# cisco/thor

Measured on AMD Instinct MI355X. Metric: encoder Mpixels/s at fixed qp, bit-exact recon vs ref, higher is better.
Workload: dtype u8

## Files before the change

### include/thor_hip.h

```cpp
#ifndef THOR_HIP_H
#define THOR_HIP_H
#include <stddef.h>
#include <stdint.h>
#ifdef __cplusplus
extern "C" {
#endif

struct thor_encoder_info;
void encode_frame_lbd(struct thor_encoder_info* encoder_info);
void encode_frame_hbd(struct thor_encoder_info* encoder_info);

typedef struct thor_hip_params {
  int width, height, qp;
  int bitdepth, input_bitdepth;
  float frame_rate;
  float lambda_coeffI, lambda_coeffP;
  float early_skip_thr;
  int enable_tb_split, enable_pb_split, max_num_ref, HQperiod;
  int num_reorder_pics, interp_ref;
  int dqpP, dqpI;
  float mqpP;
  int intra_period, intra_rdo, encoder_speed;
  int deblocking, cdef, clpf, use_block_contexts, enable_bipred;
  int cfl_intra, cfl_inter;
// ... 57 lines not shown
  int frame_type;
  int qp;
  int num_bits;
  int num_ref;
  int ref_array[4];
  int ref_frame_num[4];
  int has_sse;
  unsigned long long sse[3];
  double psnr[3];
} thor_hip_frame_stats;
int thor_hip_frame_stats_count(const thor_hip_encoder* e, int stream);
int thor_hip_get_frame_stats(const thor_hip_encoder* e, int stream, int i, thor_hip_frame_stats* out);
int thor_hip_report(const thor_hip_encoder* e, int stream, char* buf, size_t n);
int thor_hip_stat_line(const thor_hip_encoder* e, int stream, int num_frames, char* buf, size_t n);

void thor_hip_read_prof(thor_hip_encoder* e, long long out[32]);

int thor_hip_sad_batch(const uint8_t* org, int w, int h, const uint8_t* ref_plane, int plane_w, int plane_h,
                       int rstride, int bx, int by, const int* cand, int n, uint32_t* out);
int thor_hip_interp_luma(const uint8_t* ref_plane, int plane_w, int plane_h, int rstride, int pad, int bx, int by,
                         int w, int h, const int16_t* mv, int n, int bipred, uint8_t* out);
int thor_hip_code_tu_batch(const uint8_t* org, const uint8_t* pred, int size, int qp, int coeff_type, int fast, int n,
                           int16_t* coefq, uint8_t* rec, int* cbp);
typedef struct thor_hip_cell {
  int16_t mv0x, mv0y, mv1x, mv1y;
  uint8_t mode, size, tbpb, cbp;
  int8_t ref0, ref1, dir;
  uint8_t pad;
} thor_hip_cell;
int thor_hip_deblock_frame(uint8_t* yuv, int width, int height, int qp, const thor_hip_cell* cells);

int thor_hip_sad_batch_hbd(const uint16_t* org, int w, int h, const uint16_t* ref_plane, int plane_w, int plane_h,
                           int rstride, int bx, int by, const int* cand, int n, uint32_t* out);
int thor_hip_interp_luma_hbd(const uint16_t* ref_plane, int plane_w, int plane_h, int rstride, int pad, int bx, int by,
                             int w, int h, const int16_t* mv, int n, int bipred, int bitdepth, uint16_t* out);
int thor_hip_code_tu_batch_hbd(const uint16_t* org, const uint16_t* pred, int size, int qp, int coeff_type, int fast, int n,
                               int bitdepth, int16_t* coefq, uint16_t* rec, int* cbp);
int thor_hip_deblock_frame_hbd(uint16_t* yuv, int width, int height, int qp, int bitdepth, const thor_hip_cell* cells);

int thor_hip_kat_intra(const void* plane, int width, int height, int stride, int bitdepth, int size, int tb_split, int n, const int* par,
                       const void* rblocks, void* out);
int thor_hip_kat_inter_yuv(const void* yuv, int width, int height, int bitdepth, int size, int n, const int* par, const int16_t* mv, void* out);
int thor_hip_kat_average(const void* a, const void* b, int size, int bitdepth, int n, void* out);
int thor_hip_kat_cfl(const void* y, void* uv, const void* ry, int n_luma, int bitdepth, int n);
int thor_hip_kat_cdef_dir(const void* blocks, int bitdepth, int n, int* dir, int* var);
int thor_hip_kat_cdef_filter(const void* plane, int width, int height, int stride, int bitdepth, int bsize, int n, const int* par, void* out);
int thor_hip_kat_cdef_frame(int n_jobs, const void* rec_yuv, const void* org_yuv, const uint8_t* mode, int width, int height, int bitdepth, const int* qp,
                            const int* speed, const int* cdef_bits, int8_t* dir, int* var, int* fb_compact, unsigned long long* mse, int* result, int* fb_sel, void* out_yuv);
int thor_hip_kat_clpf(const void* rec_yuv, const void* org_yuv, int width, int height, int bitdepth, int qp, const thor_hip_cell* cells,
                      const int* strength, int fb_log2, const uint8_t* fb_on, uint32_t* stats, void* out_yuv);
int thor_hip_kat_interpolate(const void* yuv0, const void* yuv1, int width, int height, int bitdepth, void* out_yuv);

int thor_hip_kat_motion_estimate(const void* cur, const void* ref, int width, int height, int bitdepth, int n, const int* par, const double* lambda,
                                 const int16_t* cand, int ncand_total, int* out);
int thor_hip_kat_motion_estimate_bi(const void* cur, const void* ref0, const void* ref1, int width, int height, int bitdepth, int n, const int* par,
                                    const double* lambda, const int16_t* cand, int* out, int16_t* list_out);
int thor_hip_kat_early_skip(const int* chroma, const void* org, const void* pred, const int* size, const int* qp, const float* thr, int bitdepth, int n, int* out);
int thor_hip_kat_coeff_syntax(int n, const int* par, const int16_t* coef, int words, uint32_t* buf_single, uint32_t* buf_team, int* out);
int thor_hip_kat_block_syntax(int n, const int* par, const int16_t* pool, int npool, int words, uint32_t* buf_coop, uint32_t* buf_single, int* out);
// ... 17 lines not shown
```

### thor_amd/__init__.py

```python
from .binding import (ThorParams, Encoder, FrameLayout, lib, lib_path, load_config, sad_batch, interp_luma, code_tu_batch, deblock_frame,
                      frame_sse, frame_sse_depth, kat_depth_up, kat_depth_down, layout_bytes, kat_layout_in,
                      kat_layout_out, build_native, REPO_ROOT)

__all__ = ['ThorParams', 'Encoder', 'FrameLayout', 'lib', 'lib_path', 'load_config', 'sad_batch', 'interp_luma', 'code_tu_batch', 'deblock_frame',
           'frame_sse', 'frame_sse_depth', 'kat_depth_up', 'kat_depth_down', 'layout_bytes', 'kat_layout_in', 'kat_layout_out', 'build_native', 'REPO_ROOT']
```

### thor_amd/binding.py

```python
import ctypes as C
import os
import subprocess
import numpy as np

REPO_ROOT = os.path.dirname(os.path.dirname(os.path.abspath(__file__)))
_LIB = None


def lib_path():
    return os.environ.get('THOR_HIP_LIB') or os.path.join(REPO_ROOT, 'thor_amd', 'libthor_hip.so')


HIPCC_FLAGS = ['--offload-arch=gfx950', '-O3', '-std=c++17', '-ffp-contract=off', '-fno-strict-aliasing', '-fPIC', '-pthread']
NATIVE_SOURCES = ['thor_hip.cpp', 'thor_hip_lat.cpp', 'thor_hip_wide.cpp', 'thor_hip_katbits.cpp']


def build_native(force=False):
    csrc = os.path.join(REPO_ROOT, 'thor_amd', 'csrc')
    out = os.path.join(REPO_ROOT, 'thor_amd', 'libthor_hip.so')
    hdrs = [os.path.join(csrc, f) for f in os.listdir(csrc)]
    hdrs += [os.path.join(REPO_ROOT, 'include', f) for f in os.listdir(os.path.join(REPO_ROOT, 'include'))]
    newest = max(os.path.getmtime(h) for h in hdrs)
    if force or not os.path.exists(out) or os.path.getmtime(out) < newest:
        hipcc = '/opt/rocm/bin/hipcc' if os.path.exists('/opt/rocm/bin/hipcc') else 'hipcc'
# ... 341 lines not shown
    else:
        rc = lib().thor_hip_interp_luma(_vp(ref_padded), pic_w, pic_h, ref_padded.shape[1], pad, bx, by, w, h, _vp(mvs), len(mvs),
                                        bipred, _vp(out))
    if rc:
        raise RuntimeError(f'thor_hip_interp_luma rc={rc}')
    return out


def code_tu_batch(org, pred, qp, coeff_type, fast, bitdepth=8):
    T = _pix(bitdepth)
    org = np.ascontiguousarray(org, dtype=T); pred = np.ascontiguousarray(pred, dtype=T)
    n, size = org.shape[0], org.shape[1]
    q = min(size, 16)
    coefq = np.zeros((n, q, q), dtype=np.int16); rec = np.zeros_like(org); cbp = np.zeros(n, dtype=np.int32)
    if bitdepth > 8:
        rc = lib().thor_hip_code_tu_batch_hbd(_vp(org), _vp(pred), size, qp, coeff_type, fast, n, bitdepth, _vp(coefq), _vp(rec), _vp(cbp))
    else:
        rc = lib().thor_hip_code_tu_batch(_vp(org), _vp(pred), size, qp, coeff_type, fast, n, _vp(coefq), _vp(rec), _vp(cbp))
    if rc:
        raise RuntimeError(f'thor_hip_code_tu_batch rc={rc}')
    return coefq, rec, cbp


def deblock_frame(yuv, width, height, qp, cells, bitdepth=8):
    yuv = np.ascontiguousarray(yuv, dtype=_pix(bitdepth)).copy()
    cells = np.ascontiguousarray(cells, dtype=np.uint8)
    assert yuv.size == width * height * 3 // 2 and cells.size == (width // 4) * (height // 4) * 16
    if bitdepth > 8:
        rc = lib().thor_hip_deblock_frame_hbd(_vp(yuv), width, height, qp, bitdepth, _vp(cells))
    else:
        rc = lib().thor_hip_deblock_frame(_vp(yuv), width, height, qp, _vp(cells))
    if rc:
        raise RuntimeError(f'thor_hip_deblock_frame rc={rc}')
    return yuv


def _kat(name, *args):
    fn = getattr(lib(), name)
    fn.restype = C.c_int
    rc = fn(*args)
    if rc:
        raise RuntimeError(f'{name} rc={rc}')


def kat_intra(plane, size, par, bitdepth=8, rblocks=None):
    T = _pix(bitdepth)
# ... 205 lines not shown
```

### thor_amd/csrc/hip_kat.h

```cpp
#pragma once
#include "tk_kat_bits.h"
namespace tk {
template <typename PIX>
__global__ __launch_bounds__(64) void k_kat_sad(const PIX* org, int w, int h, const PIX* refp, int rstride, int bx, int by, const int* cand, int n,
                                               uint32_t* out) {
  const Team t = mk_team((int)threadIdx.x, 64);
  struct KC { const PIX* p; int dx, dy; };
  MeWin win;
  win.on = 0; win.w32 = nullptr; win.ox = win.oy = win.Ww = win.Wh = win.pitch = 0;
  auto cnd = [&](int c) -> KC {
    KC x;
    x.dx = cand[2 * c]; x.dy = cand[2 * c + 1];
    x.p = refp + (size_t)(by + x.dy) * rstride + bx + x.dx;
    return x;
  };
  seg_sads<SP_GLOBAL>(t, n, org, w, rstride, w, h, win, cnd, [&](int c, const KC&, int sad, int mine) { if (mine) out[c] = (uint32_t)sad; });
}
template <typename PIX>
__global__ __launch_bounds__(64) void k_kat_interp(const PIX* ref0, int rstride, int pic_w, int pic_h, int bx, int by, int w, int h,
                                                  const int16_t* mv, int bipred, int bitdepth, PIX* out) {
  const Team t = mk_team((int)threadIdx.x, 64);
  const int i = blockIdx.x;
  pred_luma<SP_GLOBAL>(t, out + (size_t)i * w * h, w, ref0 + (size_t)by * rstride + bx, rstride, w, h, mk_mv(mv[2 * i], mv[2 * i + 1]), 0,
            bipred, pic_w, pic_h, bx, by, bitdepth);
}
template <typename PIX>
__global__ __launch_bounds__(64) void k_kat_tu(const PIX* org, const PIX* pred, int size, int qp, int coeff_type, int fast, int bitdepth,
                                              int16_t* coefq, PIX* rec, int* cbp) {
  __shared__ XformWs xf;
  __shared__ XformTabs tabs;
  __shared__ int16_t cq[256];
  const Team t = mk_team((int)threadIdx.x, 64, tabs.izz);
  xf.prof = nullptr;
  xf.tabs = &tabs;
  xform_tables_fill(&tabs, (int)threadIdx.x, 64);
  t.sync();
  const int i = blockIdx.x, qs = size < 16 ? size : 16;
  const size_t o = (size_t)i * size * size;
  int c = code_tu(t, &xf, org + o, size, pred + o, size, rec + o, size, size, qp, coeff_type, fast, cq, bitdepth);
  for (int k = threadIdx.x; k < qs * qs; k += 64) coefq[(size_t)i * qs * qs + k] = cq[k];
  if (threadIdx.x == 0) cbp[i] = c;
}

template <typename PIX>
__global__ __launch_bounds__(64) void k_kat_intra(const PIX* plane, int stride, int bitdepth, int size, int tb_split, const int* par, const PIX* rblocks,
                                                 PIX* out) {
  __shared__ IntraEdge<PIX> edge;
  const Team t = mk_team((int)threadIdx.x, 64);
  const int it = blockIdx.x;
  const int* q = par + 7 * it;
  const int cbs = tb_split ? 2 * size : size;
  const PIX* rblock = tb_split ? rblocks + (size_t)it * cbs * cbs + q[5] * cbs + q[6] : nullptr;
  make_edges<SP_GLOBAL>(t, &edge, plane + (size_t)q[0] * stride + q[1], stride, rblock, cbs, q[5], q[6], q[0], q[1], size, q[2], q[3], tb_split, bitdepth);
  pred_intra<SP_GLOBAL>(t, &edge, q[0] + q[5], q[1] + q[6], size, out + (size_t)it * size * size, size, q[4], bitdepth);
}
template <typename PIX>
__global__ __launch_bounds__(kWgThreads, (sizeof(PIX) == 1 ? (int)kOcc : 2)) void k_kat_inter_yuv(Plane3<PIX> ref, int width, int height, int bitdepth, int size, const int* par, const int16_t* mv, PIX* out) {
  const Team t = mk_team((int)threadIdx.x, 64);
  const int it = blockIdx.x;
  const int* q = par + 5 * it;
  mv_t m[4];
  for (int k = 0; k < 4; k++) m[k] = mk_mv(mv[(it * 4 + k) * 2], mv[(it * 4 + k) * 2 + 1]);
  PIX* o = out + (size_t)it * (size * size * 3 / 2);
  pred_inter_yuv<SP_GLOBAL>(t, ref, o, o + size * size, o + size * size * 5 / 4, q[0], q[1], size, size, size, m, q[2], width, height, q[3], q[4], bitdepth);
// ... 159 lines not shown
  const size_t px = (size_t)n * size * size;
  const int qs = size < 16 ? size : 16;
  DevBuf<PIX> d_org(px, org), d_pred(px, pred), d_rec(px);
  DevBuf<int16_t> d_cq((size_t)n * qs * qs);
  DevBuf<int> d_cbp(n);
  hipLaunchKernelGGL(k_kat_tu<PIX>, dim3(n), dim3(64), 0, g_stream, d_org, d_pred, size, qp, coeff_type, fast, bitdepth, d_cq, d_rec,
                     d_cbp);
  HIPCHECK(hipGetLastError());
  backend::d2h(coefq, d_cq, (size_t)n * qs * qs * 2);
  backend::d2h(rec, d_rec, px * sizeof(PIX));
  backend::d2h(cbp, d_cbp, (size_t)n * 4);
  return 0;
}
extern "C" int thor_hip_code_tu_batch(const uint8_t* org, const uint8_t* pred, int size, int qp, int coeff_type, int fast, int n,
                                      int16_t* coefq, uint8_t* rec, int* cbp) {
  return kat_code_tu_batch<uint8_t>(org, pred, size, qp, coeff_type, fast, n, 8, coefq, rec, cbp);
}
extern "C" int thor_hip_code_tu_batch_hbd(const uint16_t* org, const uint16_t* pred, int size, int qp, int coeff_type, int fast, int n,
                                          int bitdepth, int16_t* coefq, uint16_t* rec, int* cbp) {
  if (bitdepth < 9 || bitdepth > 12) return 1;
  return kat_code_tu_batch<uint16_t>(org, pred, size, qp, coeff_type, fast, n, bitdepth, coefq, rec, cbp);
}

template <typename PIX> static int kat_deblock_frame(PIX* yuv, int width, int height, int qp, int bitdepth, const thor_hip_cell* cells) {
  static_assert(sizeof(thor_hip_cell) == sizeof(DbCell), "thor_hip_cell must mirror tk::DbCell");
  if (!yuv || !cells || width % 8 || height % 8 || width < 16 || height < 16 || qp < 0 || qp > 51) return 1;
  if (!ensure_init_any()) return 3;
  DevFrame<PIX> f;
  f.alloc(width, height, 0);
  DevBuf<DbCell> d_cells((size_t)(width / 4) * (height / 4), (const DbCell*)cells);
  upload_yuv(f, yuv, width, height);
  FrameJob<PIX> J;
  memset(&J, 0, sizeof(J));
  J.cfg.width = width; J.cfg.height = height; J.cfg.bitdepth = bitdepth;
  J.qp = qp; J.rec = f.p; J.cells = d_cells; J.cell_stride = width / 4;
  DevBuf<FrameJob<PIX>> d_job(1, &J);
  backend::run_deblock<PIX>(d_job, &J, 1);
  backend::dev_sync();
  download_yuv(f, yuv, width, height);
  f.release();
  return 0;
}
extern "C" int thor_hip_deblock_frame(uint8_t* yuv, int width, int height, int qp, const thor_hip_cell* cells) {
  return kat_deblock_frame<uint8_t>(yuv, width, height, qp, 8, cells);
}
extern "C" int thor_hip_deblock_frame_hbd(uint16_t* yuv, int width, int height, int qp, int bitdepth, const thor_hip_cell* cells) {
// ... 508 lines not shown
```

### thor_amd/csrc/tk_block_rd.h

```cpp
#pragma once
#include "tk_block_ctx.h"

namespace tk {
template <typename PIX> struct SsdT { typedef unsigned long long type; };
template <> struct SsdT<uint8_t> { typedef unsigned type; };
TK_DEV unsigned udot4_u8(unsigned a, unsigned b, unsigned c) {
#if TK_HOST
  for (int k = 0; k < 4; k++) c += ((a >> (8 * k)) & 0xffu) * ((b >> (8 * k)) & 0xffu);
  return c;
#else
  return __builtin_amdgcn_udot4(a, b, c, false);
#endif
}
TK_DEV unsigned udot2_u16(unsigned a, unsigned b, unsigned c) {
#if TK_HOST
  return c + (a & 0xffffu) * (b & 0xffffu) + (a >> 16) * (b >> 16);
#else
  typedef unsigned short __attribute__((ext_vector_type(2))) u16x2;
  u16x2 x, y;
  __builtin_memcpy(&x, &a, 4); __builtin_memcpy(&y, &b, 4);
  return __builtin_amdgcn_udot2(x, y, c, false);
#endif
}
template <int SP, typename PIX, int NW> TK_DEV unsigned ssd_rows(const Team t, const PIX* a_, int as, const PIX* b_, int bs, int w, int h) {
// ... 218 lines not shown
  pc->ssd_y = (long long)ssd;
  const int coeff_type = (p.mode == M_INTRA) << 1;
  int bits = 0;
  if (!tb_split) {
    pc->ybits[0] = cbp_y ? coeff_bits_team<SP_LDS>(t, ws->coef_y, size, coeff_type) : 0;
    bits = pc->ybits[0];
  } else {
    const int qy = size / 2 < kMaxQuant ? size / 2 : kMaxQuant;
    for (int tu = 0; tu < 4; tu++) {
      pc->ybits[tu] = ((cbp_y >> (3 - tu)) & 1) ? coeff_bits_team<SP_LDS>(t, ws->coef_y + tu * qy * qy, size / 2, coeff_type) : 0;
      bits += pc->ybits[tu];
    }
  }
  pc->have_ybits = 1;
  unsigned long long lb = (ssd >> (J.cfg.bitdepth * 2 - 16)) + (unsigned long long)(long long)mul_add_nofma(pc->lambda, (double)(bits + pc->head_bits), 0.5);
  if (lb > (1ull << 30)) lb = 1ull << 30;
#if TK_HOST
  { extern long long g_prune_stat[8]; g_prune_stat[p.mode == M_INTRA ? 0 : 2] += 1; if (prune_hit(pc, lb)) g_prune_stat[p.mode == M_INTRA ? 1 : 3] += 1; }
#endif
  if (team_bcast0(t, prune_hit(pc, lb))) { pc->pruned = 1; return 1; }
  return 0;
}

template <typename PIX, int SP, int SC>
TK_DEV int code_inter_plane(const Team t, JobR<PIX> J, WsP<PIX> ws, const PIX* org, int ostride,
                            const PIX* pred, PIX* rec, int size, int qp, int coeff_type, int tb_split, int16_t* coef,
                            int nd_size = 0, PruneCtx* pc = nullptr) {
  const int bd = J.cfg.bitdepth;
  if (!tb_split) {
    int fast = (size == 64 && J.cfg.encoder_speed > 0) || J.cfg.encoder_speed > 1;
    return code_tu_sp<PIX, SP, SC>(t, ws->xfp, org, ostride, pred, size, rec, size, size, qp, coeff_type, fast, coef, bd);
  }
  const int s2 = size / 2;
  int cbp = 0, index = 0;
  for (int i = 0; i < size; i += s2)
    for (int j = 0; j < size; j += s2) {
      int fast = size == 64 || J.cfg.encoder_speed > 1;
      int bit = code_tu_sp<PIX, SP, SC>(t, ws->xfp, org + i * ostride + j, ostride, pred + i * size + j, size, rec + i * size + j, size,
                        s2, qp, coeff_type, fast, coef + index, bd);
      cbp = (cbp << 1) + bit;
      if (nd_size && prune_after_quadrant<PIX, SP>(t, J, ws, nd_size, 0, (i ? 2 : 0) + (j ? 1 : 0), i, j, s2, bit, coef + index, pc)) return cbp;
      index += tmin(s2, 16) * tmin(s2, 16);
    }
  return cbp;
}

template <typename PIX, int SP>
TK_DEVNI int encode_block(const Team t, JobR<PIX> J, WsP<PIX> ws, Node& nd_, BlkParam& p, BitSink& bs,
                          int reuse_pred = 0, PruneCtx* pc = nullptr) {
  const auto& c = J.cfg;
  const NodePos nd = node_pos(&nd_);
  const int size = nd.size, sizeC = size >> 1;
  const int yc = nd.ypos >> 1, xc = nd.xpos >> 1;
  const int qpY = TKU(J.qp), qpC = TK_TAB.chroma_qp[qpY];
  const int tb_split = TKU(p.tb_param) > 0 ? TKU(p.tb_param) : 0;
  const int zero_block = TKU(p.tb_param) == -1;
  const int ftI = (TKU(J.frame_type) == F_I) << 1;
  const int bd = TKU(c.bitdepth);
  p.tb_split = (int8_t)tb_split;
  const int bigc = SP == SP_GLOBAL && tb_split && sizeC >= 32;
  ws->coef_u = bigc ? ws->coef_u_big : ws->coef_u_small;
  ws->coef_v = bigc ? ws->coef_v_big : ws->coef_v_small;
  const PIX* oy = ws->org_y;
  const PIX* ou = ws->org_u;
  const PIX* ov = ws->org_v;
  const int osy = TKU(ws->org_sy), osc = TKU(ws->org_sc);
  int cbp_y = 0, cbp_u = 0, cbp_v = 0;
// ... 22 lines not shown
      make_edges<SP>(t, ws->edgep, fy, J.rec.sy, (const PIX*)nullptr, 0, 0, 0, nd.ypos, nd.xpos, size, ur, dl, 0, bd);
      pred_intra<SP>(t, ws->edgep, nd.ypos, nd.xpos, size, ws->pred_y, size, p.intra_mode, bd);
      t.sync();
      cbp_y = code_tu_sp<PIX, SP, SP_LDS>(t, ws->xfp, oy, osy, ws->pred_y, size, ws->rec_y, size, size, qpY, ftI | 0,
                      c.encoder_speed > 1, ws->coef_y, bd);
    }
    if (prune_after_luma<PIX, SP>(t, J, ws, size, nd.bw, nd.bh, p, cbp_y, tb_split, pc)) return 0;
    const int csplit = tb_split && sizeC > 4;
    if (csplit) {
      const int s2 = sizeC / 2;
      int index = 0;
      for (int i = 0; i < sizeC; i += s2)
        for (int j = 0; j < sizeC; j += s2) {
          make_edges<SP>(t, ws->edgep, fu, J.rec.sc, ws->rec_u + i * sizeC + j, sizeC, i, j, yc, xc, s2, ur, dl, 1, bd);
          pred_intra<SP>(t, ws->edgep, yc + i, xc + j, s2, ws->pred_u + i * sizeC + j, sizeC, p.intra_mode, bd);
          t.sync();
          make_edges<SP>(t, ws->edgep, fv, J.rec.sc, ws->rec_v + i * sizeC + j, sizeC, i, j, yc, xc, s2, ur, dl, 1, bd);
          pred_intra<SP>(t, ws->edgep, yc + i, xc + j, s2, ws->pred_v + i * sizeC + j, sizeC, p.intra_mode, bd);
          t.sync();
          if (c.cfl_intra)
            improve_uv<PIX, SP>(t, ws, ws->pred_y + i * sizeC + j, ws->pred_u + i * sizeC + j, ws->pred_v + i * sizeC + j,
                       ws->rec_y + (i << 1) * size + (j << 1), s2 << 1, sizeC << 1, size, bd);
          int bu, bv;
          if (bigc) {
            bu = code_tu_sp<PIX, SP, SP_GLOBAL>(t, ws->xfp, ou + i * osc + j, osc, ws->pred_u + i * sizeC + j, sizeC,
                             ws->rec_u + i * sizeC + j, sizeC, s2, qpC, ftI | 1, c.encoder_speed > 1, ws->coef_u + index, bd);
            bv = code_tu_sp<PIX, SP, SP_GLOBAL>(t, ws->xfp, ov + i * osc + j, osc, ws->pred_v + i * sizeC + j, sizeC,
                             ws->rec_v + i * sizeC + j, sizeC, s2, qpC, ftI | 1, c.encoder_speed > 1, ws->coef_v + index, bd);
          } else {
            bu = code_tu_sp<PIX, SP, SP_LDS>(t, ws->xfp, ou + i * osc + j, osc, ws->pred_u + i * sizeC + j, sizeC,
                             ws->rec_u + i * sizeC + j, sizeC, s2, qpC, ftI | 1, c.encoder_speed > 1, ws->coef_u + index, bd);
            bv = code_tu_sp<PIX, SP, SP_LDS>(t, ws->xfp, ov + i * osc + j, osc, ws->pred_v + i * sizeC + j, sizeC,
                             ws->rec_v + i * sizeC + j, sizeC, s2, qpC, ftI | 1, c.encoder_speed > 1, ws->coef_v + index, bd);
          }
          cbp_u = (cbp_u << 1) + bu;
          cbp_v = (cbp_v << 1) + bv;
          index += tmin(s2, 16) * tmin(s2, 16);
        }
    } else {
      make_edges<SP>(t, ws->edgep, fu, J.rec.sc, (const PIX*)nullptr, 0, 0, 0, yc, xc, sizeC, ur, dl, 0, bd);
      pred_intra<SP>(t, ws->edgep, yc, xc, sizeC, ws->pred_u, sizeC, p.intra_mode, bd);
      t.sync();
      make_edges<SP>(t, ws->edgep, fv, J.rec.sc, (const PIX*)nullptr, 0, 0, 0, yc, xc, sizeC, ur, dl, 0, bd);
      pred_intra<SP>(t, ws->edgep, yc, xc, sizeC, ws->pred_v, sizeC, p.intra_mode, bd);
      t.sync();
      if (c.cfl_intra) improve_uv<PIX, SP>(t, ws, ws->pred_y, ws->pred_u, ws->pred_v, ws->rec_y, size, size, size, bd);
      cbp_u = code_tu_sp<PIX, SP, SP_LDS>(t, ws->xfp, ou, osc, ws->pred_u, sizeC, ws->rec_u, sizeC, sizeC, qpC, ftI | 1,
                      c.encoder_speed > 1, ws->coef_u, bd);
      cbp_v = code_tu_sp<PIX, SP, SP_LDS>(t, ws->xfp, ov, osc, ws->pred_v, sizeC, ws->rec_v, sizeC, sizeC, qpC, ftI | 1,
                      c.encoder_speed > 1, ws->coef_v, bd);
    }
  } else {
    const int split = (TKU(p.mode) == M_INTER || TKU(p.mode) == M_BIPRED) ? c.enable_pb_split : 0;
    if (!(reuse_pred == 2 || (reuse_pred && !c.cfl_inter))) predict_inter<PIX, SP>(t, J, ws, nd_, p, split);
    if (TKU(p.mode) == M_SKIP || zero_block) {
      copy_block<SP, SP>(t, ws->rec_y, size, ws->pred_y, size, nd.bw, nd.bh);
      copy_block<SP, SP>(t, ws->rec_u, sizeC, ws->pred_u, sizeC, nd.bw >> 1, nd.bh >> 1);
      copy_block<SP, SP>(t, ws->rec_v, sizeC, ws->pred_v, sizeC, nd.bw >> 1, nd.bh >> 1);
      t.sync();
    } else {
      cbp_y = code_inter_plane<PIX, SP, SP_LDS>(t, J, ws, oy, osy, ws->pred_y, ws->rec_y, size, qpY, ftI | 0, tb_split, ws->coef_y, size, pc);
      if (prune_after_luma<PIX, SP>(t, J, ws, size, nd.bw, nd.bh, p, cbp_y, tb_split, pc)) return 0;
      if (c.cfl_inter) improve_uv<PIX, SP>(t, ws, ws->pred_y, ws->pred_u, ws->pred_v, ws->rec_y, size, size, size, bd);
      const int csplit = tb_split && sizeC > 4;
      if (bigc) {
        cbp_u = code_inter_plane<PIX, SP, SP_GLOBAL>(t, J, ws, ou, osc, ws->pred_u, ws->rec_u, sizeC, qpC, ftI | 1, csplit, ws->coef_u);
        cbp_v = code_inter_plane<PIX, SP, SP_GLOBAL>(t, J, ws, ov, osc, ws->pred_v, ws->rec_v, sizeC, qpC, ftI | 1, csplit, ws->coef_v);
      } else {
        cbp_u = code_inter_plane<PIX, SP, SP_LDS>(t, J, ws, ou, osc, ws->pred_u, ws->rec_u, sizeC, qpC, ftI | 1, csplit, ws->coef_u);
        cbp_v = code_inter_plane<PIX, SP, SP_LDS>(t, J, ws, ov, osc, ws->pred_v, ws->rec_v, sizeC, qpC, ftI | 1, csplit, ws->coef_v);
      }
    }
  }
  p.cbp_y = (uint8_t)cbp_y;
  p.cbp_u = (uint8_t)cbp_u;
  p.cbp_v = (uint8_t)cbp_v;
  TK_PROF_T0();
  const SynCtx syn = lds_ld(&nd_.syn);
  const int* yb = (pc && pc->have_ybits) ? pc->ybits : nullptr;
  int nb_ = bigc ? bs_block_t<false, SP_GLOBAL>(bs, syn, p, ws->coef_y, ws->coef_u, ws->coef_v, &t, yb)
                 : bs_block_t<false, SP_LDS>(bs, syn, p, ws->coef_y, ws->coef_u, ws->coef_v, &t, yb);
  TK_PROF_ADD(ws, PF_BITS);
  return nb_;
}

template <typename PIX, int SP>
TK_DEV unsigned rdo_trial(const Team t, JobR<PIX> J, WsP<PIX> ws, Node& nd, BlkParam& p, double lambda,
                          int reuse_pred = 0, unsigned prune_thr = 0xffffffffu, const unsigned long long* bestkey = nullptr,
                          unsigned order = 0, int* nbits_out = nullptr, int* untouched = nullptr) {
  BitSink cnt;
  cnt.buf = nullptr; cnt.pos = 0; cnt.cap = 0; cnt.emit = 0; cnt.ovf = 0;
  PruneCtx pc;
  pc.thr = prune_thr; pc.bestkey = bestkey; pc.order = order; pc.lambda = lambda; pc.ssd_y = -1; pc.have_ybits = 0; pc.pruned = 0; pc.ssd_part = 0; pc.bits_part = 0;
// ... 44 lines not shown
```

### thor_amd/csrc/tk_xform.h

```cpp
#pragma once
#include "tk_common.h"

#ifndef TK_PROF_T0
#if TK_PROF_MACROS
#ifdef THOR_PROF_WALL
#define TK_CYC() ((long long)wall_clock64())
#else
#define TK_CYC() ((long long)__builtin_readcyclecounter())
#endif
#define TK_PROF_T0() long long pt0_ = TK_CYC()
#define TK_PROF_ADD(ws, id) do { if (t.rank == 0) (ws)->prof[id] += TK_CYC() - pt0_; } while (0)
#define TK_PROF_MARK(v) long long v = TK_CYC()
#define TK_PROF_ACC(ws, id, v) do { if (t.rank == 0) (ws)->prof[id] += TK_CYC() - (v); } while (0)
#define TK_PROF_CNT(ws, id) do { if (t.rank == 0) (ws)->prof[id] += 1; } while (0)
#else
#define TK_PROF_T0() do {} while (0)
#define TK_PROF_ADD(ws, id) do {} while (0)
#define TK_PROF_MARK(v) do {} while (0)
#define TK_PROF_ACC(ws, id, v) do {} while (0)
#define TK_PROF_CNT(ws, id) do {} while (0)
#endif
#endif

namespace tk {

struct XformTabs {
  alignas(16) int16_t dct32[1024];
  int16_t izz[336];
  alignas(16) int16_t dctT[1360];
};
static_assert(offsetof(XformTabs, izz) == 1024 * sizeof(int16_t), "dct32 must directly precede izz");
static_assert(offsetof(XformTabs, dctT) == (1024 + 336) * sizeof(int16_t), "dctT must directly follow izz");
#if TK_HOST
#define TK_DCT32(t, ws) ((ws)->tabs->dct32)
#define TK_DCTT(t, ws) ((ws)->tabs->dctT)
#else
#define TK_DCT32(t, ws) (TK_LDS_PTR((t).izz) - 1024)
#define TK_DCTT(t, ws) (TK_LDS_PTR((t).izz) + 336)
#endif
TK_DEV int dctT_off(int n) { return n == 32 ? 0 : n == 16 ? 1024 : n == 8 ? 1280 : 1344; }
struct XformWs {
  int flag;
  long long* prof;
// ... 414 lines not shown
    dequantize<SC>(t, ws, coefq, qp, size);
    inv_transform_recon<PIX, SP>(t, ws, pred, pstride, rec, rstride, size, bitdepth);
    TK_PROF_ACC(ws, 31, pi0_);
  } else {
    copy_block<SP, SP>(t, rec, rstride, pred, pstride, size, size);
    t.sync();
  }
#if !defined(THOR_PROF_ME) && !defined(THOR_PROF_MD)
  TK_PROF_ADD(ws, (size <= 4 ? 16 : size == 8 ? 17 : size == 16 ? 18 : size == 32 ? 19 : 20));
  TK_PROF_CNT(ws, (size <= 4 ? 21 : size == 8 ? 22 : size == 16 ? 23 : size == 32 ? 24 : 25));
#endif
  TK_PROF_ADD(ws, 6);
  return cbp;
}
template <typename PIX>
TK_DEV int code_tu(const Team t, XformWs* ws, const PIX* org, int ostride, const PIX* pred, int pstride, PIX* rec,
                   int rstride, int size, int qp, int coeff_type, int fast, int16_t* coefq, int bitdepth) {
  const int lb = tk_uniform(tk_is_lds(pred)), lc = tk_uniform(tk_is_lds(coefq));
  if (lb) return code_tu_sp<PIX, SP_LDS, SP_LDS>(t, ws, org, ostride, pred, pstride, rec, rstride, size, qp, coeff_type, fast, coefq, bitdepth);
  if (lc) return code_tu_sp<PIX, SP_GLOBAL, SP_LDS>(t, ws, org, ostride, pred, pstride, rec, rstride, size, qp, coeff_type, fast, coefq, bitdepth);
  return code_tu_sp<PIX, SP_GLOBAL, SP_GLOBAL>(t, ws, org, ostride, pred, pstride, rec, rstride, size, qp, coeff_type, fast, coefq, bitdepth);
}

}
```

Before: 163.7.

## Batch small 4x4/8x8 transform units into one grouped team transform-quant pass

Adds code_tu_group, which runs forward DCT, RDOQ-style quantization, dequant and inverse transform for up to eight small TUs at once across the 64-lane team, using a pointer table stored in LDS. Split luma TUs, chroma U/V pairs and split chroma quads in inter and intra coding now go through it instead of one TU at a time. The goal is to fill idle lanes and cut the number of team syncs when blocks are small. In exchange it reimplements the quant and transform paths, which must stay bit-exact with code_tu_sp. It also adds a standalone test kernel and host binding.

```diff
diff --git a/include/thor_hip.h b/include/thor_hip.h
--- a/include/thor_hip.h
+++ b/include/thor_hip.h
@@ -103,6 +103,8 @@
                          int w, int h, const int16_t* mv, int n, int bipred, uint8_t* out);
 int thor_hip_code_tu_batch(const uint8_t* org, const uint8_t* pred, int size, int qp, int coeff_type, int fast, int n,
                            int16_t* coefq, uint8_t* rec, int* cbp);
+int thor_hip_code_tu_group(const uint8_t* org, const uint8_t* pred, int size, int G, int qp, int coeff_type, int fast, int n, int in_lds,
+                           int16_t* coefq, uint8_t* rec, int* cbp);
 typedef struct thor_hip_cell {
   int16_t mv0x, mv0y, mv1x, mv1y;
   uint8_t mode, size, tbpb, cbp;
@@ -116,6 +118,8 @@
 int thor_hip_interp_luma_hbd(const uint16_t* ref_plane, int plane_w, int plane_h, int rstride, int pad, int bx, int by,
                              int w, int h, const int16_t* mv, int n, int bipred, int bitdepth, uint16_t* out);
 int thor_hip_code_tu_batch_hbd(const uint16_t* org, const uint16_t* pred, int size, int qp, int coeff_type, int fast, int n,
+                               int bitdepth, int16_t* coefq, uint16_t* rec, int* cbp);
+int thor_hip_code_tu_group_hbd(const uint16_t* org, const uint16_t* pred, int size, int G, int qp, int coeff_type, int fast, int n, int in_lds,
                                int bitdepth, int16_t* coefq, uint16_t* rec, int* cbp);
 int thor_hip_deblock_frame_hbd(uint16_t* yuv, int width, int height, int qp, int bitdepth, const thor_hip_cell* cells);
 
diff --git a/thor_amd/__init__.py b/thor_amd/__init__.py
--- a/thor_amd/__init__.py
+++ b/thor_amd/__init__.py
@@ -1,6 +1,6 @@
-from .binding import (ThorParams, Encoder, FrameLayout, lib, lib_path, load_config, sad_batch, interp_luma, code_tu_batch, deblock_frame,
+from .binding import (ThorParams, Encoder, FrameLayout, lib, lib_path, load_config, sad_batch, interp_luma, code_tu_batch, code_tu_group, deblock_frame,
                       frame_sse, frame_sse_depth, kat_depth_up, kat_depth_down, layout_bytes, kat_layout_in,
                       kat_layout_out, build_native, REPO_ROOT)
 
-__all__ = ['ThorParams', 'Encoder', 'FrameLayout', 'lib', 'lib_path', 'load_config', 'sad_batch', 'interp_luma', 'code_tu_batch', 'deblock_frame',
+__all__ = ['ThorParams', 'Encoder', 'FrameLayout', 'lib', 'lib_path', 'load_config', 'sad_batch', 'interp_luma', 'code_tu_batch', 'code_tu_group', 'deblock_frame',
            'frame_sse', 'frame_sse_depth', 'kat_depth_up', 'kat_depth_down', 'layout_bytes', 'kat_layout_in', 'kat_layout_out', 'build_native', 'REPO_ROOT']
diff --git a/thor_amd/binding.py b/thor_amd/binding.py
--- a/thor_amd/binding.py
+++ b/thor_amd/binding.py
@@ -387,6 +387,21 @@
     return coefq, rec, cbp
 
 
+def code_tu_group(org, pred, qp, coeff_type, fast, bitdepth=8, in_lds=0):
+    T = _pix(bitdepth)
+    org = np.ascontiguousarray(org, dtype=T); pred = np.ascontiguousarray(pred, dtype=T)
+    n, G, size = org.shape[0], org.shape[1], org.shape[2]
+    assert org.shape == pred.shape == (n, G, size, size)
+    coefq = np.zeros((n, G, size, size), dtype=np.int16); rec = np.zeros_like(org); cbp = np.zeros((n, G), dtype=np.int32)
+    if bitdepth > 8:
+        rc = lib().thor_hip_code_tu_group_hbd(_vp(org), _vp(pred), size, G, qp, coeff_type, fast, n, in_lds, bitdepth, _vp(coefq), _vp(rec), _vp(cbp))
+    else:
+        rc = lib().thor_hip_code_tu_group(_vp(org), _vp(pred), size, G, qp, coeff_type, fast, n, in_lds, _vp(coefq), _vp(rec), _vp(cbp))
+    if rc:
+        raise RuntimeError(f'thor_hip_code_tu_group rc={rc}')
+    return coefq, rec, cbp
+
+
 def deblock_frame(yuv, width, height, qp, cells, bitdepth=8):
     yuv = np.ascontiguousarray(yuv, dtype=_pix(bitdepth)).copy()
     cells = np.ascontiguousarray(cells, dtype=np.uint8)
diff --git a/thor_amd/csrc/hip_kat.h b/thor_amd/csrc/hip_kat.h
--- a/thor_amd/csrc/hip_kat.h
+++ b/thor_amd/csrc/hip_kat.h
@@ -40,6 +40,39 @@
   int c = code_tu(t, &xf, org + o, size, pred + o, size, rec + o, size, size, qp, coeff_type, fast, cq, bitdepth);
   for (int k = threadIdx.x; k < qs * qs; k += 64) coefq[(size_t)i * qs * qs + k] = cq[k];
   if (threadIdx.x == 0) cbp[i] = c;
+}
+template <typename PIX>
+__global__ __launch_bounds__(kWgThreads, (sizeof(PIX) == 1 ? (int)kOcc : 2)) void k_kat_tu_group(const PIX* org, const PIX* pred, int size, int G, int qp, int coeff_type, int fast,
+                                                                                                 int bitdepth, int in_lds, int16_t* coefq, PIX* rec, int* cbp) {
+  __shared__ XformWs xf;
+  __shared__ XformTabs tabs;
+  __shared__ int16_t cq[kTuGroupEntries];
+  __shared__ alignas(16) PIX sb[3 * kTuGroupEntries];
+  const int lane = (int)threadIdx.x;
+  const Team t = mk_team(lane, 64, tabs.izz);
+  xf.prof = nullptr;
+  xf.tabs = &tabs;
+  xform_tables_fill(&tabs, lane, 64);
+  const int N = size * size, row = G * size;
+  const size_t o = (size_t)blockIdx.x * G * N;
+  if (in_lds)
+    for (int k = lane; k < G * N; k += 64) {
+      const int u = k / N, e = k % N, at = (e / size) * row + u * size + e % size;
+      sb[at] = org[o + k]; sb[kTuGroupEntries + at] = pred[o + k];
+    }
+  __syncthreads();
+  for (int u = 0; u < G; u++) {
+    if (in_lds) tu_group_set<PIX>(t, &xf, u, sb + u * size, sb + kTuGroupEntries + u * size, sb + 2 * kTuGroupEntries + u * size, cq + u * N);
+    else tu_group_set<PIX>(t, &xf, u, org + o + u * N, pred + o + u * N, rec + o + u * N, cq + u * N);
+  }
+  const int m = in_lds ? code_tu_group<PIX, SP_LDS, SP_LDS>(t, &xf, G, row, row, row, size, qp, coeff_type, fast, bitdepth)
+                       : code_tu_group<PIX, SP_GLOBAL, SP_LDS>(t, &xf, G, size, size, size, size, qp, coeff_type, fast, bitdepth);
+  __syncthreads();
+  for (int k = lane; k < G * N; k += 64) {
+    coefq[o + k] = cq[k];
+    if (in_lds) rec[o + k] = sb[2 * kTuGroupEntries + ((k % N) / size) * row + (k / N) * size + k % size];
+  }
+  if (lane < G) cbp[(size_t)blockIdx.x * G + lane] = (m >> lane) & 1;
 }
 
 template <typename PIX>
@@ -245,6 +278,33 @@
   return kat_code_tu_batch<uint16_t>(org, pred, size, qp, coeff_type, fast, n, bitdepth, coefq, rec, cbp);
 }
 
+template <typename PIX>
+static int kat_code_tu_group(const PIX* org, const PIX* pred, int size, int G, int qp, int coeff_type, int fast, int n, int in_lds, int bitdepth,
+                             int16_t* coefq, PIX* rec, int* cbp) {
+  if (!org || !pred || !coefq || !rec || !cbp || n <= 0 || qp < 0 || qp > 51 || (in_lds != 0 && in_lds != 1)) return 1;
+  if ((size != 4 && size != 8) || G < 1 || G > tk::kTuGroupMax || G * size * size > tk::kTuGroupEntries) return 2;
+  if (!ensure_init_any()) return 3;
+  const size_t px = (size_t)n * G * size * size;
+  DevBuf<PIX> d_org(px, org), d_pred(px, pred), d_rec(px);
+  DevBuf<int16_t> d_cq(px);
+  DevBuf<int> d_cbp((size_t)n * G);
+  hipLaunchKernelGGL(k_kat_tu_group<PIX>, dim3(n), dim3(64), 0, g_stream, d_org, d_pred, size, G, qp, coeff_type, fast, bitdepth, in_lds, d_cq, d_rec, d_cbp);
+  HIPCHECK(hipGetLastError());
+  backend::d2h(coefq, d_cq, px * 2);
+  backend::d2h(rec, d_rec, px * sizeof(PIX));
+  backend::d2h(cbp, d_cbp, (size_t)n * G * 4);
+  return 0;
+}
+extern "C" int thor_hip_code_tu_group(const uint8_t* org, const uint8_t* pred, int size, int G, int qp, int coeff_type, int fast, int n, int in_lds,
+                                      int16_t* coefq, uint8_t* rec, int* cbp) {
+  return kat_code_tu_group<uint8_t>(org, pred, size, G, qp, coeff_type, fast, n, in_lds, 8, coefq, rec, cbp);
+}
+extern "C" int thor_hip_code_tu_group_hbd(const uint16_t* org, const uint16_t* pred, int size, int G, int qp, int coeff_type, int fast, int n, int in_lds,
+                                          int bitdepth, int16_t* coefq, uint16_t* rec, int* cbp) {
+  if (bitdepth < 9 || bitdepth > 12) return 1;
+  return kat_code_tu_group<uint16_t>(org, pred, size, G, qp, coeff_type, fast, n, in_lds, bitdepth, coefq, rec, cbp);
+}
+
 template <typename PIX> static int kat_deblock_frame(PIX* yuv, int width, int height, int qp, int bitdepth, const thor_hip_cell* cells) {
   static_assert(sizeof(thor_hip_cell) == sizeof(DbCell), "thor_hip_cell must mirror tk::DbCell");
   if (!yuv || !cells || width % 8 || height % 8 || width < 16 || height < 16 || qp < 0 || qp > 51) return 1;
diff --git a/thor_amd/csrc/tk_block_rd.h b/thor_amd/csrc/tk_block_rd.h
--- a/thor_amd/csrc/tk_block_rd.h
+++ b/thor_amd/csrc/tk_block_rd.h
@@ -264,6 +264,32 @@
   return 0;
 }
 
+#ifndef TK_TU_GROUP_Y
+#define TK_TU_GROUP_Y 8
+#endif
+#ifndef TK_TU_GROUP_C
+#define TK_TU_GROUP_C 8
+#endif
+TK_DEV int tu_group_cbp4(int m) { return ((m & 1) << 3) | ((m & 2) << 1) | ((m & 4) >> 1) | ((m & 8) >> 3); }
+
+template <typename PIX, int SP>
+TK_DEV int prune_after_group(const Team t, JobR<PIX> J, WsP<PIX> ws, int nd_size, int s2, int cbp, const int16_t* coef, PruneCtx* pc) {
+  if (!prune_active(pc)) return 0;
+  pc->ssd_part += (long long)ssd_total(t, ssd_part<SP>(t, ws->org_y, ws->org_sy, ws->rec_y, nd_size, nd_size, nd_size));
+  for (int tu = 0; tu < 4; tu++) {
+    pc->ybits[tu] = ((cbp >> (3 - tu)) & 1) ? coeff_bits_team<SP_LDS>(t, coef + tu * s2 * s2, s2, 0) : 0;
+    pc->bits_part += pc->ybits[tu];
+  }
+  pc->ssd_y = pc->ssd_part; pc->have_ybits = 1;
+  unsigned long long lb = ((unsigned long long)pc->ssd_part >> (J.cfg.bitdepth * 2 - 16)) + (unsigned long long)(long long)mul_add_nofma(pc->lambda, (double)(pc->bits_part + pc->head_bits), 0.5);
+  if (lb > (1ull << 30)) lb = 1ull << 30;
+#if TK_HOST
+  { extern long long g_prune_stat[8]; g_prune_stat[4] += 1; if (prune_hit(pc, lb)) g_prune_stat[6] += 1; }
+#endif
+  if (team_bcast0(t, prune_hit(pc, lb))) { pc->pruned = 1; return 1; }
+  return 0;
+}
+
 template <typename PIX, int SP, int SC>
 TK_DEV int code_inter_plane(const Team t, JobR<PIX> J, WsP<PIX> ws, const PIX* org, int ostride,
                             const PIX* pred, PIX* rec, int size, int qp, int coeff_type, int tb_split, int16_t* coef,
@@ -274,6 +300,17 @@
     return code_tu_sp<PIX, SP, SC>(t, ws->xfp, org, ostride, pred, size, rec, size, size, qp, coeff_type, fast, coef, bd);
   }
   const int s2 = size / 2;
+  if constexpr (SC == SP_LDS) {
+    if (s2 <= (nd_size ? TK_TU_GROUP_Y : TK_TU_GROUP_C)) {
+      for (int tu = 0; tu < 4; tu++) {
+        const int i = (tu >> 1) * s2, j = (tu & 1) * s2;
+        tu_group_set<PIX>(t, ws->xfp, tu, org + i * ostride + j, pred + i * size + j, rec + i * size + j, coef + tu * s2 * s2);
+      }
+      const int cbp = tu_group_cbp4(code_tu_group<PIX, SP, SC>(t, ws->xfp, 4, ostride, size, size, s2, qp, coeff_type, J.cfg.encoder_speed > 1, bd));
+      if (nd_size) prune_after_group<PIX, SP>(t, J, ws, nd_size, s2, cbp, coef, pc);
+      return cbp;
+    }
+  }
   int cbp = 0, index = 0;
   for (int i = 0; i < size; i += s2)
     for (int j = 0; j < size; j += s2) {
@@ -285,6 +322,32 @@
       index += tmin(s2, 16) * tmin(s2, 16);
     }
   return cbp;
+}
+
+template <typename PIX, int SP>
+TK_DEV void code_inter_chroma(const Team t, JobR<PIX> J, WsP<PIX> ws, const PIX* ou, const PIX* ov, int osc, int sizeC, int qp, int coeff_type,
+                              int csplit, int& cbp_u, int& cbp_v) {
+  const int bd = J.cfg.bitdepth, fast = J.cfg.encoder_speed > 1;
+  const int s2 = sizeC / 2;
+  if (!csplit && sizeC <= TK_TU_GROUP_C) {
+    tu_group_set<PIX>(t, ws->xfp, 0, ou, ws->pred_u, ws->rec_u, ws->coef_u);
+    tu_group_set<PIX>(t, ws->xfp, 1, ov, ws->pred_v, ws->rec_v, ws->coef_v);
+    const int m = code_tu_group<PIX, SP, SP_LDS>(t, ws->xfp, 2, osc, sizeC, sizeC, sizeC, qp, coeff_type, fast, bd);
+    cbp_u = m & 1; cbp_v = m >> 1;
+    return;
+  }
+  if (csplit && s2 <= TK_TU_GROUP_C && 8 * s2 * s2 <= kTuGroupEntries) {
+    for (int tu = 0; tu < 4; tu++) {
+      const int i = (tu >> 1) * s2, j = (tu & 1) * s2;
+      tu_group_set<PIX>(t, ws->xfp, tu, ou + i * osc + j, ws->pred_u + i * sizeC + j, ws->rec_u + i * sizeC + j, ws->coef_u + tu * s2 * s2);
+      tu_group_set<PIX>(t, ws->xfp, 4 + tu, ov + i * osc + j, ws->pred_v + i * sizeC + j, ws->rec_v + i * sizeC + j, ws->coef_v + tu * s2 * s2);
+    }
+    const int m = code_tu_group<PIX, SP, SP_LDS>(t, ws->xfp, 8, osc, sizeC, sizeC, s2, qp, coeff_type, fast, bd);
+    cbp_u = tu_group_cbp4(m & 15); cbp_v = tu_group_cbp4(m >> 4);
+    return;
+  }
+  cbp_u = code_inter_plane<PIX, SP, SP_LDS>(t, J, ws, ou, osc, ws->pred_u, ws->rec_u, sizeC, qp, coeff_type, csplit, ws->coef_u);
+  cbp_v = code_inter_plane<PIX, SP, SP_LDS>(t, J, ws, ov, osc, ws->pred_v, ws->rec_v, sizeC, qp, coeff_type, csplit, ws->coef_v);
 }
 
 template <typename PIX, int SP>
@@ -353,7 +416,12 @@
             improve_uv<PIX, SP>(t, ws, ws->pred_y + i * sizeC + j, ws->pred_u + i * sizeC + j, ws->pred_v + i * sizeC + j,
                        ws->rec_y + (i << 1) * size + (j << 1), s2 << 1, sizeC << 1, size, bd);
           int bu, bv;
-          if (bigc) {
+          if (!bigc && s2 <= TK_TU_GROUP_C) {
+            tu_group_set<PIX>(t, ws->xfp, 0, ou + i * osc + j, ws->pred_u + i * sizeC + j, ws->rec_u + i * sizeC + j, ws->coef_u + index);
+            tu_group_set<PIX>(t, ws->xfp, 1, ov + i * osc + j, ws->pred_v + i * sizeC + j, ws->rec_v + i * sizeC + j, ws->coef_v + index);
+            const int m = code_tu_group<PIX, SP, SP_LDS>(t, ws->xfp, 2, osc, sizeC, sizeC, s2, qpC, ftI | 1, c.encoder_speed > 1, bd);
+            bu = m & 1; bv = m >> 1;
+          } else if (bigc) {
             bu = code_tu_sp<PIX, SP, SP_GLOBAL>(t, ws->xfp, ou + i * osc + j, osc, ws->pred_u + i * sizeC + j, sizeC,
                              ws->rec_u + i * sizeC + j, sizeC, s2, qpC, ftI | 1, c.encoder_speed > 1, ws->coef_u + index, bd);
             bv = code_tu_sp<PIX, SP, SP_GLOBAL>(t, ws->xfp, ov + i * osc + j, osc, ws->pred_v + i * sizeC + j, sizeC,
@@ -376,10 +444,17 @@
       pred_intra<SP>(t, ws->edgep, yc, xc, sizeC, ws->pred_v, sizeC, p.intra_mode, bd);
       t.sync();
       if (c.cfl_intra) improve_uv<PIX, SP>(t, ws, ws->pred_y, ws->pred_u, ws->pred_v, ws->rec_y, size, size, size, bd);
-      cbp_u = code_tu_sp<PIX, SP, SP_LDS>(t, ws->xfp, ou, osc, ws->pred_u, sizeC, ws->rec_u, sizeC, sizeC, qpC, ftI | 1,
-                      c.encoder_speed > 1, ws->coef_u, bd);
-      cbp_v = code_tu_sp<PIX, SP, SP_LDS>(t, ws->xfp, ov, osc, ws->pred_v, sizeC, ws->rec_v, sizeC, sizeC, qpC, ftI | 1,
-                      c.encoder_speed > 1, ws->coef_v, bd);
+      if (sizeC <= TK_TU_GROUP_C) {
+        tu_group_set<PIX>(t, ws->xfp, 0, ou, ws->pred_u, ws->rec_u, ws->coef_u);
+        tu_group_set<PIX>(t, ws->xfp, 1, ov, ws->pred_v, ws->rec_v, ws->coef_v);
+        const int m = code_tu_group<PIX, SP, SP_LDS>(t, ws->xfp, 2, osc, sizeC, sizeC, sizeC, qpC, ftI | 1, c.encoder_speed > 1, bd);
+        cbp_u = m & 1; cbp_v = m >> 1;
+      } else {
+        cbp_u = code_tu_sp<PIX, SP, SP_LDS>(t, ws->xfp, ou, osc, ws->pred_u, sizeC, ws->rec_u, sizeC, sizeC, qpC, ftI | 1,
+                        c.encoder_speed > 1, ws->coef_u, bd);
+        cbp_v = code_tu_sp<PIX, SP, SP_LDS>(t, ws->xfp, ov, osc, ws->pred_v, sizeC, ws->rec_v, sizeC, sizeC, qpC, ftI | 1,
+                        c.encoder_speed > 1, ws->coef_v, bd);
+      }
     }
   } else {
     const int split = (TKU(p.mode) == M_INTER || TKU(p.mode) == M_BIPRED) ? c.enable_pb_split : 0;
@@ -398,8 +473,7 @@
         cbp_u = code_inter_plane<PIX, SP, SP_GLOBAL>(t, J, ws, ou, osc, ws->pred_u, ws->rec_u, sizeC, qpC, ftI | 1, csplit, ws->coef_u);
         cbp_v = code_inter_plane<PIX, SP, SP_GLOBAL>(t, J, ws, ov, osc, ws->pred_v, ws->rec_v, sizeC, qpC, ftI | 1, csplit, ws->coef_v);
       } else {
-        cbp_u = code_inter_plane<PIX, SP, SP_LDS>(t, J, ws, ou, osc, ws->pred_u, ws->rec_u, sizeC, qpC, ftI | 1, csplit, ws->coef_u);
-        cbp_v = code_inter_plane<PIX, SP, SP_LDS>(t, J, ws, ov, osc, ws->pred_v, ws->rec_v, sizeC, qpC, ftI | 1, csplit, ws->coef_v);
+        code_inter_chroma<PIX, SP>(t, J, ws, ou, ov, osc, sizeC, qpC, ftI | 1, csplit, cbp_u, cbp_v);
       }
     }
   }
diff --git a/thor_amd/csrc/tk_xform.h b/thor_amd/csrc/tk_xform.h
--- a/thor_amd/csrc/tk_xform.h
+++ b/thor_amd/csrc/tk_xform.h
@@ -13,12 +13,14 @@
 #define TK_PROF_MARK(v) long long v = TK_CYC()
 #define TK_PROF_ACC(ws, id, v) do { if (t.rank == 0) (ws)->prof[id] += TK_CYC() - (v); } while (0)
 #define TK_PROF_CNT(ws, id) do { if (t.rank == 0) (ws)->prof[id] += 1; } while (0)
+#define TK_PROF_CNTN(ws, id, n) do { if (t.rank == 0) (ws)->prof[id] += (n); } while (0)
 #else
 #define TK_PROF_T0() do {} while (0)
 #define TK_PROF_ADD(ws, id) do {} while (0)
 #define TK_PROF_MARK(v) do {} while (0)
 #define TK_PROF_ACC(ws, id, v) do {} while (0)
 #define TK_PROF_CNT(ws, id) do {} while (0)
+#define TK_PROF_CNTN(ws, id, n) do {} while (0)
 #endif
 #endif
 
@@ -479,4 +481,197 @@
   return code_tu_sp<PIX, SP_GLOBAL, SP_GLOBAL>(t, ws, org, ostride, pred, pstride, rec, rstride, size, qp, coeff_type, fast, coefq, bitdepth);
 }
 
-}
+template <typename PIX> struct TuUnit {
+  const PIX* org;
+  const PIX* pred;
+  PIX* rec;
+  int16_t* coefq;
+};
+enum { kTuGroupMax = 8, kTuGroupEntries = 256, kTuGroupTab = 32 * 32 - kTuGroupMax * 16 };
+static_assert(sizeof(TuUnit<uint8_t>) == 32 && sizeof(TuUnit<uint16_t>) == 32, "eight units of four pointers in 256 bytes");
+static_assert(kTuGroupTab >= kTuGroupEntries && kTuGroupTab % 8 == 0, "the pointer table lies behind the group's residuals / inverse stage-1 values, 16-byte aligned");
+template <typename PIX> TK_DEV TuUnit<PIX>* tu_group_tab(XformWs* ws) { return (TuUnit<PIX>*)(void*)(ws->in + kTuGroupTab); }
+template <typename PIX> TK_DEV void tu_group_set(const Team t, XformWs* ws, int u, const PIX* org, const PIX* pred, PIX* rec, int16_t* coefq) {
+  if (t.rank == 0) {
+    TuUnit<PIX> e;
+    e.org = org; e.pred = pred; e.rec = rec; e.coefq = coefq;
+    lds_st(tu_group_tab<PIX>(ws) + u, e);
+  }
+}
+template <int SP, typename PIX> TK_DEV void load4(const PIX* p, int vec, int* out) {
+  if (vec) { load_samples<SP, PIX, 4>(p, out); return; }
+  const auto q = spc<SP>(p);
+  for (int k = 0; k < 4; k++) out[k] = (int)q[k];
+}
+template <int SP, typename PIX> TK_DEV void store4(PIX* p, int vec, const int* in) {
+  if (vec) { store_samples<SP, PIX, 4>(p, in); return; }
+  const auto q = spc<SP>(p);
+  for (int k = 0; k < 4; k++) q[k] = (PIX)in[k];
+}
+
+template <typename PIX, int SP, int SC>
+TK_DEVNI int code_tu_group(const Team t, XformWs* ws, int G, int ostride, int pstride, int rstride, int size, int qp, int coeff_type, int fast,
+                           int bitdepth) {
+  ws = tk_uniform_ptr(ws); G = tk_uniform(G); ostride = tk_uniform(ostride); pstride = tk_uniform(pstride); rstride = tk_uniform(rstride);
+  size = tk_uniform(size); qp = tk_uniform(qp); coeff_type = tk_uniform(coeff_type); bitdepth = tk_uniform(bitdepth);
+  (void)fast;
+  TK_PROF_T0();
+  const int lgs = ilog2((unsigned)size), lgN = 2 * lgs, N = 1 << lgN, total = G << lgN;
+  const int ppr = size >> 2, lgp = lgs - 2, lgu = lgN - 2, pieces = G << lgu;
+  const auto tab = ldsc(tu_group_tab<PIX>(ws));
+  lds_i16* const in = TK_LDS_PTR(ws->in);
+  lds_i16* const tmp = TK_LDS_PTR(ws->tmp);
+  lds_i16* const coef = TK_LDS_PTR(ws->coef);
+  const lds_i16* const dct = TK_DCT32(t, ws);
+  const int rs = 5 - lgs;
+  const int S = (int)sizeof(PIX);
+  t.sync();
+  int vec;
+  {
+    unsigned al = (unsigned)(ostride * S) | (unsigned)(pstride * S) | (unsigned)(rstride * S);
+    for (int k = t.rank; k < G; k += t.size) al |= (unsigned)(uintptr_t)tab[k].org | (unsigned)(uintptr_t)tab[k].pred | (unsigned)(uintptr_t)tab[k].rec;
+#ifdef TK_NOVEC
+    al = 1u;
+#endif
+    vec = team_ballot(t, (al & (unsigned)(4 * S - 1)) != 0) == 0ull;
+  }
+  for (int k = t.rank; k < pieces; k += t.size) {
+    const int u = k >> lgu, e = k & ((1 << lgu) - 1), i = e >> lgp, j = (e & (ppr - 1)) << 2;
+    int o[4], p[4];
+    load4<SP, PIX>(tab[u].org + i * ostride + j, vec, o);
+    load4<SP, PIX>(tab[u].pred + i * pstride + j, vec, p);
+    int16_t r4[4];
+    for (int q = 0; q < 4; q++) r4[q] = (int16_t)(o[q] - p[q]);
+#if TK_HOST
+    __builtin_memcpy(ws->in + (u << lgN) + i * size + j, r4, 8);
+#else
+    typedef uint32_t __attribute__((ext_vector_type(2))) v2;
+    v2 x;
+    __builtin_memcpy(&x, r4, 8);
+    *(TK_LDS v2*)(in + (u << lgN) + i * size + j) = x;
+#endif
+  }
+  t.sync();
+  {
+    const int shift_1 = lgs + bitdepth - 8, add_1 = 1 << (shift_1 - 1), shift_2 = lgs + 5, add_2 = 1 << (shift_2 - 1);
+    for (int k = t.rank; k < total; k += t.size) {
+      const int ub = k & ~(N - 1), e = k & (N - 1), i = e >> lgs, j = e & (size - 1);
+      const int sum = dot_i16(dct + ((i << rs) << 5), in + ub + j * size, size, 0);
+      tmp[ub + i * size + j] = (int16_t)((sum + add_1) >> shift_1);
+    }
+    t.sync();
+    for (int k = t.rank; k < total; k += t.size) {
+      const int ub = k & ~(N - 1), e = k & (N - 1), i = e >> lgs, j = e & (size - 1);
+      const int sum = dot_i16(dct + ((i << rs) << 5), tmp + ub + j * size, size, 0);
+      coef[ub + i * size + j] = (int16_t)((sum + add_2) >> shift_2);
+    }
+    t.sync();
+  }
+  TK_PROF_ADD(ws, 30);
+  TK_PROF_MARK(pq0_);
+  int cbpm = 0;
+  {
+    const int intra_block = (coeff_type >> 1) & 1;
+    const IzzRef izzr = izz_ref(t, size);
+    const int scale = quant_scale(qp % 6);
+    const int shift2 = 21 - lgs + qp / 6;
+    const int offl = intra_block ? (38 << (shift2 - 8)) : -(26 << (shift2 - 8));
+    const int off0 = (intra_block ? 102 : 51) << (shift2 - 8);
+    const int off1 = (intra_block ? 115 : 90) << (shift2 - 8);
+    const int W = t.size, seg = W < N ? W : N, chunk = W > N ? W : N;
+    const int lo = t.rank & ~(seg - 1), sr = t.rank - lo;
+    const unsigned long long smask = (seg >= 64 ? ~0ull : ((1ull << seg) - 1ull)) << lo;
+    for (int cb = 0; cb < total; cb += chunk) {
+      const int ub = cb + (W > N ? lo : 0), u = ub >> lgN, valid = ub < total;
+      const auto cq = spc<SC>(tab[valid ? u : 0].coefq);
+      int last_pos = -1;
+      for (int r = 0; r < N; r += seg) {
+        const int p = r + sr;
+        int nz = 0;
+        if (valid) {
+          const int l = iabs((int)coef[ub + izzr.z[p]]) * scale + offl;
+          nz = ((l > 0 ? l : -l) >> shift2) != 0;
+        }
+        const unsigned long long m = team_ballot(t, nz) & smask;
+        if (m) last_pos = r + top_set(m) - lo;
+      }
+      int carry = 1, any = 0;
+      for (int r = 0; r < N; r += seg) {
+        const int p = r + sr;
+        const int active = valid && p <= last_pos;
+        int c = 0, lev0 = 0, lev1 = 0;
+        if (active) {
+          c = coef[ub + izzr.z[p]];
+          const int ac = scale * iabs(c);
+          const int level0 = ac >> shift2;
+          lev1 = (ac + (level0 > 0 ? off1 : off0)) >> shift2;
+          lev0 = (ac + (level0 > 1 ? off1 : off0)) >> shift2;
+        }
+        const int to0 = active && lev1 == 0, to1 = active && lev0 > 1;
+        const unsigned long long mK = team_ballot(t, to0 || to1) & smask, mV = team_ballot(t, to1);
+        const int j = prev_set(mK, t.rank);
+        const int mode = j < 0 ? carry : (int)((mV >> j) & 1ull);
+        const int lev = mode ? lev1 : lev0;
+        if (valid) cq[izzr.z[p]] = (int16_t)(c < 0 ? -lev : lev);
+        any |= (team_ballot(t, active && lev != 0) & smask) != 0ull;
+        const int jj = top_set(mK);
+        if (jj >= 0) carry = (int)((mV >> jj) & 1ull);
+      }
+      const unsigned long long mb = team_ballot(t, any && sr == 0);
+      for (int q = 0; q < chunk; q += N)
+        if ((mb >> (W > N ? q : 0)) & 1ull) cbpm |= 1 << ((cb + q) >> lgN);
+    }
+    cbpm = tk_uniform(cbpm);
+    t.sync();
+  }
+  TK_PROF_ACC(ws, 12, pq0_);
+  TK_PROF_MARK(pi0_);
+  const lds_i16* const mt = TK_DCTT(t, ws) + dctT_off(size);
+  if (cbpm) {
+    const int lshift = qp / 6, rshift = lgs - 1;
+    const int64_t dscale = dequant_scale(qp % 6);
+    for (int k = t.rank; k < total; k += t.size) {
+      const int u = k >> lgN, e = k & (N - 1);
+      if (!((cbpm >> u) & 1)) continue;
+      const int64_t c = spc<SC>(tab[u].coefq)[e];
+      int16_t r;
+      if (lshift >= rshift) r = (int16_t)((c * dscale) << (lshift - rshift));
+      else r = (int16_t)((c * dscale + ((int64_t)1 << (rshift - lshift - 1))) >> (rshift - lshift));
+      coef[(u << lgN) + ((e & (size - 1)) << lgs) + (e >> lgs)] = r;
+    }
+    t.sync();
+    for (int k = t.rank; k < total; k += t.size) {
+      const int u = k >> lgN, ub = k & ~(N - 1), e = k & (N - 1), i = e >> lgs, j = e & (size - 1);
+      if (!((cbpm >> u) & 1)) continue;
+      const int sum = dot_i16(mt + j * size, coef + ub + i * size, size, 0);
+      in[ub + j * size + i] = (int16_t)clampi((sum + 64) >> 7, -32768, 32767);
+    }
+    t.sync();
+  }
+  {
+    const int shift_2 = 20 - bitdepth, add_2 = 1 << (shift_2 - 1);
+    for (int k = t.rank; k < pieces; k += t.size) {
+      const int u = k >> lgu, e = k & ((1 << lgu) - 1), i = e >> lgp, j = (e & (ppr - 1)) << 2;
+      int p[4];
+      load4<SP, PIX>(tab[u].pred + i * pstride + j, vec, p);
+      if ((cbpm >> u) & 1) {
+        TK_UNROLL
+        for (int q = 0; q < 4; q++) {
+          const int sum = dot_i16(mt + (j + q) * size, in + (u << lgN) + i * size, size, 0);
+          p[q] = sat_pix(clampi((sum + add_2) >> shift_2, -32768, 32767) + p[q], bitdepth);
+        }
+      }
+      store4<SP, PIX>(tab[u].rec + i * rstride + j, vec, p);
+    }
+    t.sync();
+  }
+  TK_PROF_ACC(ws, 31, pi0_);
+#if !defined(THOR_PROF_ME) && !defined(THOR_PROF_MD)
+  TK_PROF_ADD(ws, (size <= 4 ? 16 : 17));
+  TK_PROF_CNTN(ws, (size <= 4 ? 21 : 22), G);
+#endif
+  TK_PROF_ADD(ws, 6);
+  return cbpm;
+}
+
+}
```

Result: no change. 164.5 (median of 6 runs) (+0.5%).
